# zju-pi/diff-sampler

Measured on AMD Instinct MI355X. Metric: images/sec (whole node) at NFE=10, EDM CIFAR-10, higher is better.
Workload: dtype fp32; 1 GPU; EDM CIFAR-10 32x32 SongUNet (55.7M params), DPM-Solver++(2M) logSNR NFE=10, batch 256/GPU; launch=eager

## Files before the change

### diff_sampler_amd/csrc/conv3x3_thin.hip

```cpp
#include "igemm_common.h"

namespace igemm {
namespace {

template <int CTRL>
__device__ __forceinline__ float thin_dpp_add(float v) {
    return v + __builtin_bit_cast(float, __builtin_amdgcn_update_dpp(0, __builtin_bit_cast(int, v), CTRL, 0xf, 0xf, false));
}

template <int NORM, bool UPD>
__global__ void __launch_bounds__(256, 4) conv3x3_thin_kernel(const KParams p, const ds_update_args u) {
    extern __shared__ __attribute__((aligned(16))) float smem_thin[];
    f32x4* wl = reinterpret_cast<f32x4*>(smem_thin);
    const int tid = threadIdx.x, lane = tid & 63, wave = tid >> 6;
    const int C = p.c0, S = C / 32;
    for (int i = tid; i < 9 * S * 32; i += 256) {
        const int j = i & 7, q = (i >> 3) & 3, rest = i >> 5;
        const int tap = rest / S, step = rest - tap * S;
        const float* b = p.b + (size_t)(step * 9 + tap) * 32 + j * 4 + q;
        wl[i] = f32x4{b[0], b[(size_t)p.ldb], b[2 * (size_t)p.ldb], b[3 * (size_t)p.ldb]};
    }
    __syncthreads();
    const int R = p.mtiles;
    const int mb = blockIdx.x * (32 * R) + wave * (8 * R);
    if (mb >= p.M) return;
    const int img = mb / p.HW;
    const int g = lane >> 3, j = lane & 7;
    const float* coef = NORM ? p.norm + (size_t)img * 3 * C + j * 4 : nullptr;
    const float scale = p.scale;
    f32x4 bias = {0.f, 0.f, 0.f, 0.f};
    if (p.colbias) {
#pragma unroll
        for (int n = 0; n < 4; ++n) bias[n] = n < p.N ? p.colbias[n] : 0.f;
    }
#pragma unroll 1
    for (int round = 0; round < R; ++round) {
        const int m = mb + round * 8 + g;
        const int pim = m - img * p.HW;
        const int y = pim / p.W, x = pim - y * p.W;
        const float* src[9]; float keep[9];
#pragma unroll
        for (int t = 0; t < 9; ++t) {
            const int yy = y + t / 3 - 1, xx = x + t % 3 - 1;
            const bool ok = (unsigned)yy < (unsigned)p.H && (unsigned)xx < (unsigned)p.W;
            src[t] = p.a0 + (size_t)(ok ? (img * p.H + yy) * p.W + xx : m) * p.lda0 + j * 4;
            keep[t] = ok ? 1.f : 0.f;
        }
        f32x4 acc = {0.f, 0.f, 0.f, 0.f};
#pragma unroll 1
        for (int s = 0; s < S; ++s) {
            f32x4 mu = {0.f, 0.f, 0.f, 0.f}, ga = mu, be = mu;
            if constexpr (NORM) {
                mu = *reinterpret_cast<const f32x4*>(coef + s * 32);
                ga = *reinterpret_cast<const f32x4*>(coef + C + s * 32);
                be = *reinterpret_cast<const f32x4*>(coef + 2 * C + s * 32);
            }
            constexpr int TG = NORM ? 3 : 9;
#pragma unroll
            for (int t0 = 0; t0 < 9; t0 += TG) {
                f32x4 v[TG];
#pragma unroll
                for (int t = 0; t < TG; ++t) v[t] = *reinterpret_cast<const f32x4*>(src[t0 + t] + s * 32);
#pragma unroll
                for (int t = 0; t < TG; ++t) {
                    f32x4 a = v[t];
                    if constexpr (NORM) {
                        a = (a - mu) * ga + be;
                        if constexpr (NORM == 2) {
#pragma unroll
                            for (int e = 0; e < 4; ++e) a[e] = ds_silu(a[e]);
                        }
                    }
                    a *= keep[t0 + t];
                    const f32x4* wp = wl + (((t0 + t) * S + s) * 4) * 8 + j;
                    acc += a[0] * wp[0] + a[1] * wp[8] + a[2] * wp[16] + a[3] * wp[24];
                }
            }
        }
#pragma unroll
        for (int n = 0; n < 4; ++n) {
            float r = acc[n];
            r = thin_dpp_add<0xB1>(r);
            r = thin_dpp_add<0x4E>(r);
            r = thin_dpp_add<0x141>(r);
            acc[n] = r;
        }
        if (j == 0) {
            DsUpdCoefs k{};
            float cskip = 0.f, cout_ = 0.f;
            if constexpr (UPD) {
                k = ds_upd_load_coefs(u, img);
                cskip = ds_c_skip(k.sig, u.sigma_data); cout_ = ds_c_out(k.sig, u.sigma_data);
            }
#pragma unroll
            for (int n = 0; n < 4; ++n) {
                if (n < p.N) {
                    const float o = (acc[n] + bias[n]) * scale;
                    if (p.out_planar) p.out[((size_t)img * p.N + n) * p.HW + pim] = o;
                    else p.out[(size_t)m * p.ldo + n] = o;
                    if constexpr (UPD) {
                        const size_t off = ((size_t)img * p.N + n) * p.HW + pim;
                        const float x = u.xe[off];
                        const float xb = u.xb != u.xe ? u.xb[off] : x;
                        float mm, xo;
                        ds_upd_element(k, cskip, cout_, true, u.store_d != 0, x, xb, o, u.hist[0] != nullptr, u.hist[0] ? u.hist[0][off] : 0.f,
                                       u.hist[1] != nullptr, u.hist[1] ? u.hist[1][off] : 0.f, u.hist[2] != nullptr, u.hist[2] ? u.hist[2][off] : 0.f, mm, xo);
                        if (u.m_out) u.m_out[off] = mm;
                        if (u.x_out) u.x_out[off] = xo;
                    }
                }
            }
        }
    }
}

}

bool conv3x3_thin_applicable(const KParams& p) {
    if (p.taps != 9 || p.stride > 1 || p.N < 1 || p.N > 4) return false;
    if (p.c0 <= 0 || p.c0 % 32 || p.c1 || p.ec0 || p.ec1) return false;
    if (p.HW != p.H * p.W || p.HW % 64 || p.M % 64) return false;
    if (p.res || p.cbias || p.rowbias || p.stats || p.act != DS_ACT_NONE || p.splits > 1) return false;
    if (p.norm && p.norm_act != DS_ACT_NONE && p.norm_act != DS_ACT_SILU) return false;
    if (p.nrows_b < 4) return false;
    if (9 * p.c0 * 16 > 150 * 1024) return false;
    return true;
}

static bool thin_update_on(const KParams& p) { return p.upd && (p.upd->x_out || p.upd->m_out); }

int conv3x3_thin_check_update(const KParams& p) {
    if (!thin_update_on(p)) return DS_OK;
    const ds_update_args& u = *p.upd;
    if (!p.out_planar || !u.xe || !u.xb || !u.raw || u.afs || u.f_ld != 0) return DS_E_ARG;
    if (u.c != p.N || (long long)u.n * u.h * u.w != (long long)p.M || u.h * u.w != p.HW) return DS_E_ARG;
    if (u.coefs && u.coef_rows != 1 && u.coef_rows != u.n) return DS_E_ARG;
    return DS_OK;
}

int launch_conv3x3_thin(KParams& p, hipStream_t stream) {
    const int smem = 9 * p.c0 * 16;
    int rounds = 8;
    while (rounds > 1 && (p.M + 32 * rounds - 1) / (32 * rounds) < 512) rounds >>= 1;
    p.mtiles = rounds;
    const unsigned blocks = (unsigned)((p.M + 32 * rounds - 1) / (32 * rounds));
    const bool upd = thin_update_on(p);
    ds_update_args u{};
    if (upd) u = *p.upd;
#define DST_LAUNCH(NORM_, UPD_)                                                                                    \
    do {                                                                                                           \
        DS_ENSURE_DYN_LDS((&conv3x3_thin_kernel<NORM_, UPD_>), 160 * 1024);                                        \
        hipLaunchKernelGGL((conv3x3_thin_kernel<NORM_, UPD_>), dim3(blocks), dim3(256), smem, stream, p, u);       \
    } while (0)
    if (p.norm && p.norm_act == DS_ACT_SILU) { if (upd) DST_LAUNCH(2, true); else DST_LAUNCH(2, false); }
    else if (p.norm) { if (upd) DST_LAUNCH(1, true); else DST_LAUNCH(1, false); }
    else { if (upd) DST_LAUNCH(0, true); else DST_LAUNCH(0, false); }
#undef DST_LAUNCH
    DS_CHECK_LAUNCH();
    return DS_OK;
}

}
```

Baseline: 513.2 images/sec.

## Stage activated input halo tile in LDS for thin 3x3 conv with prefetch

Restructures the thin-output 3x3 conv kernel so each block loads its input tile plus halo once per 32-channel step into LDS. The norm/SiLU activation is applied once per staged element instead of once per tap, and the next step's global loads are prefetched into registers while the current step computes. The round count becomes a template parameter, so accumulators for all rounds stay in registers. Previously each pixel reloaded and re-normalized its nine neighbours from global memory. In exchange it needs more LDS, lowers launch bounds occupancy from 4 to 2 blocks, adds two barriers per channel step, and adds geometry code that must handle row and image boundaries, including a slower fallback when a tile spans two images.

```diff
diff --git a/diff_sampler_amd/csrc/conv3x3_thin.hip b/diff_sampler_amd/csrc/conv3x3_thin.hip
--- a/diff_sampler_amd/csrc/conv3x3_thin.hip
+++ b/diff_sampler_amd/csrc/conv3x3_thin.hip
@@ -8,82 +8,165 @@
     return v + __builtin_bit_cast(float, __builtin_amdgcn_update_dpp(0, __builtin_bit_cast(int, v), CTRL, 0xf, 0xf, false));
 }
 
-template <int NORM, bool UPD>
-__global__ void __launch_bounds__(256, 4) conv3x3_thin_kernel(const KParams p, const ds_update_args u) {
+constexpr int THIN_NI = 12;
+
+__host__ __device__ inline void thin_geometry(int H, int W, int R, int& nc, int& narrow, int& cells) {
+    const int TP = 32 * R, HW = H * W;
+    const int rows = TP % W == 0 ? TP / W : W % TP == 0 ? 1 : (TP + W - 2) / W + 1;
+    const int imgs = HW % TP == 0 ? 1 : TP % HW == 0 ? TP / HW : (TP + HW - 2) / HW + 1;
+    narrow = W % TP == 0 && W > TP;
+    nc = narrow ? TP + 2 : W + 2;
+    cells = (rows + 2 * imgs) * nc;
+}
+
+template <int NORM, bool UPD, int R>
+__global__ void __launch_bounds__(256, 2) conv3x3_thin_kernel(const KParams p, const ds_update_args u) {
     extern __shared__ __attribute__((aligned(16))) float smem_thin[];
-    f32x4* wl = reinterpret_cast<f32x4*>(smem_thin);
     const int tid = threadIdx.x, lane = tid & 63, wave = tid >> 6;
     const int C = p.c0, S = C / 32;
+    f32x4* wl = reinterpret_cast<f32x4*>(smem_thin);
+    f32x4* hal = wl + 9 * S * 32;
+    const int g = lane >> 3, j = lane & 7;
+    constexpr int TP = 32 * R;
+    const int NC = p.WP, HP2 = p.H + 2;
+    const int mb0 = blockIdx.x * TP;
+    const int mlast = (mb0 + TP < p.M ? mb0 + TP : p.M) - 1;
+    const int img0 = mb0 / p.HW, imgL = mlast / p.HW;
+    const int pim0 = mb0 - img0 * p.HW, y0 = pim0 / p.W, x0 = pim0 - y0 * p.W;
+    const int yL = (mlast - imgL * p.HW) / p.W;
+    const int cb = p.nimg ? x0 - 1 : -1;
+    const int prb = img0 * HP2 + y0;
+    const int nitems = (imgL * HP2 + yL + 3 - prb) * NC * 8;
+    const bool multi = imgL != img0;
+    const int pb = mb0 - x0 - p.W;
+    const float* a_base = p.a0 + (long long)pb * p.lda0;
+    auto item_src = [&](int it, unsigned& off, int& im) __attribute__((always_inline)) {
+        const int cell = it >> 3, row = cell / NC, col = cell - row * NC;
+        const int pr = prb + row;
+        im = pr / HP2;
+        const int yy = pr - im * HP2 - 1, xx = cb + col;
+        const bool ok = it < nitems && (unsigned)yy < (unsigned)p.H && (unsigned)xx < (unsigned)p.W;
+        off = (unsigned)(((ok ? (im * p.H + yy) * p.W + xx : mb0) - pb) * p.lda0 + j * 4);
+        return ok;
+    };
+    auto load_quad = [&](unsigned off, int s) __attribute__((always_inline)) {
+        return *reinterpret_cast<const f32x4*>(reinterpret_cast<const char*>(a_base + s * 32) + (size_t)(off * 4u));
+    };
+    unsigned off[THIN_NI], okm = 0;
+#pragma unroll
+    for (int i = 0; i < THIN_NI; ++i) {
+        int im;
+        if (item_src(i * 256 + tid, off[i], im)) okm |= 1u << i;
+    }
+    f32x4 v[THIN_NI];
+    f32x4 mu = {0.f, 0.f, 0.f, 0.f}, ga = mu, be = mu;
+    auto load_coefs = [&](int im, int s) __attribute__((always_inline)) {
+        if constexpr (NORM) {
+            const float* cf = p.norm + (size_t)im * 3 * C + j * 4 + s * 32;
+            mu = *reinterpret_cast<const f32x4*>(cf);
+            ga = *reinterpret_cast<const f32x4*>(cf + C);
+            be = *reinterpret_cast<const f32x4*>(cf + 2 * C);
+        }
+    };
+    auto prefetch = [&](int s) __attribute__((always_inline)) {
+        if (multi) return;
+#pragma unroll
+        for (int i = 0; i < THIN_NI; ++i)
+            if (i * 256 < nitems) v[i] = load_quad(off[i], s);
+        load_coefs(img0, s);
+    };
+    auto activate = [&](f32x4 a) __attribute__((always_inline)) {
+        if constexpr (NORM) {
+            a = (a - mu) * ga + be;
+            if constexpr (NORM == 2) {
+#pragma unroll
+                for (int e = 0; e < 4; ++e) a[e] = ds_silu(a[e]);
+            }
+        }
+        return a;
+    };
+    const f32x4 zero4 = {0.f, 0.f, 0.f, 0.f};
+    auto stage = [&](int s) __attribute__((always_inline)) {
+        DS_RACE_SKEW(wave);
+        if (!multi) {
+#pragma unroll
+            for (int i = 0; i < THIN_NI; ++i) {
+                if (i * 256 >= nitems) break;
+                const int it = i * 256 + tid;
+                const f32x4 a = activate(v[i]);
+                if (it < nitems) hal[it] = (okm >> i) & 1u ? a : zero4;
+            }
+        }
+        for (int it = (multi ? 0 : THIN_NI * 256) + tid; it < nitems; it += 256) {
+            unsigned o_; int im;
+            const bool ok = item_src(it, o_, im);
+            const f32x4 a = load_quad(o_, s);
+            if (multi) load_coefs(im, s);
+            hal[it] = ok ? activate(a) : zero4;
+        }
+    };
+    prefetch(0);
+    DS_RACE_SKEW(wave);
     for (int i = tid; i < 9 * S * 32; i += 256) {
-        const int j = i & 7, q = (i >> 3) & 3, rest = i >> 5;
+        const int jj = i & 7, q = (i >> 3) & 3, rest = i >> 5;
         const int tap = rest / S, step = rest - tap * S;
-        const float* b = p.b + (size_t)(step * 9 + tap) * 32 + j * 4 + q;
+        const float* b = p.b + (size_t)(step * 9 + tap) * 32 + jj * 4 + q;
         wl[i] = f32x4{b[0], b[(size_t)p.ldb], b[2 * (size_t)p.ldb], b[3 * (size_t)p.ldb]};
     }
-    __syncthreads();
-    const int R = p.mtiles;
-    const int mb = blockIdx.x * (32 * R) + wave * (8 * R);
-    if (mb >= p.M) return;
-    const int img = mb / p.HW;
-    const int g = lane >> 3, j = lane & 7;
-    const float* coef = NORM ? p.norm + (size_t)img * 3 * C + j * 4 : nullptr;
+    const int mbw = mb0 + wave * (8 * R);
+    const bool active = mbw < p.M;
+    int cc[R];
+#pragma unroll
+    for (int r = 0; r < R; ++r) {
+        const int m = active ? mbw + r * 8 + g : mb0;
+        const int img = m / p.HW, pim = m - img * p.HW, y = pim / p.W, x = pim - y * p.W;
+        cc[r] = ((img * HP2 + y + 1 - prb) * NC + (x - cb)) * 8 + j;
+    }
+    f32x4 acc[R];
+#pragma unroll
+    for (int r = 0; r < R; ++r) acc[r] = zero4;
+#pragma unroll 1
+    for (int s = 0; s < S; ++s) {
+        stage(s);
+        __syncthreads();
+        if (s + 1 < S) prefetch(s + 1);
+        if (active) {
+#pragma unroll
+            for (int t = 0; t < 9; ++t) {
+                const f32x4* wp = wl + ((t * S + s) * 4) * 8 + j;
+                const f32x4 w0 = wp[0], w1 = wp[8], w2 = wp[16], w3 = wp[24];
+                const int d = ((t / 3 - 1) * NC + (t % 3 - 1)) * 8;
+constexpr int RG = R < 4 ? R : 4;
+#pragma unroll
+                for (int r0 = 0; r0 < R; r0 += RG) {
+                    f32x4 a[RG];
+#pragma unroll
+                    for (int r = 0; r < RG; ++r) a[r] = hal[cc[r0 + r] + d];
+#pragma unroll
+                    for (int r = 0; r < RG; ++r) acc[r0 + r] += a[r][0] * w0 + a[r][1] * w1 + a[r][2] * w2 + a[r][3] * w3;
+                }
+            }
+        }
+        if (s + 1 < S) __syncthreads();
+    }
+    if (!active) return;
     const float scale = p.scale;
-    f32x4 bias = {0.f, 0.f, 0.f, 0.f};
+    f32x4 bias = zero4;
     if (p.colbias) {
 #pragma unroll
         for (int n = 0; n < 4; ++n) bias[n] = n < p.N ? p.colbias[n] : 0.f;
     }
-#pragma unroll 1
-    for (int round = 0; round < R; ++round) {
-        const int m = mb + round * 8 + g;
-        const int pim = m - img * p.HW;
-        const int y = pim / p.W, x = pim - y * p.W;
-        const float* src[9]; float keep[9];
-#pragma unroll
-        for (int t = 0; t < 9; ++t) {
-            const int yy = y + t / 3 - 1, xx = x + t % 3 - 1;
-            const bool ok = (unsigned)yy < (unsigned)p.H && (unsigned)xx < (unsigned)p.W;
-            src[t] = p.a0 + (size_t)(ok ? (img * p.H + yy) * p.W + xx : m) * p.lda0 + j * 4;
-            keep[t] = ok ? 1.f : 0.f;
-        }
-        f32x4 acc = {0.f, 0.f, 0.f, 0.f};
-#pragma unroll 1
-        for (int s = 0; s < S; ++s) {
-            f32x4 mu = {0.f, 0.f, 0.f, 0.f}, ga = mu, be = mu;
-            if constexpr (NORM) {
-                mu = *reinterpret_cast<const f32x4*>(coef + s * 32);
-                ga = *reinterpret_cast<const f32x4*>(coef + C + s * 32);
-                be = *reinterpret_cast<const f32x4*>(coef + 2 * C + s * 32);
-            }
-            constexpr int TG = NORM ? 3 : 9;
-#pragma unroll
-            for (int t0 = 0; t0 < 9; t0 += TG) {
-                f32x4 v[TG];
-#pragma unroll
-                for (int t = 0; t < TG; ++t) v[t] = *reinterpret_cast<const f32x4*>(src[t0 + t] + s * 32);
-#pragma unroll
-                for (int t = 0; t < TG; ++t) {
-                    f32x4 a = v[t];
-                    if constexpr (NORM) {
-                        a = (a - mu) * ga + be;
-                        if constexpr (NORM == 2) {
-#pragma unroll
-                            for (int e = 0; e < 4; ++e) a[e] = ds_silu(a[e]);
-                        }
-                    }
-                    a *= keep[t0 + t];
-                    const f32x4* wp = wl + (((t0 + t) * S + s) * 4) * 8 + j;
-                    acc += a[0] * wp[0] + a[1] * wp[8] + a[2] * wp[16] + a[3] * wp[24];
-                }
-            }
-        }
+#pragma unroll
+    for (int r = 0; r < R; ++r) {
+        const int m = mbw + r * 8 + g;
+        const int img = m / p.HW, pim = m - img * p.HW;
 #pragma unroll
         for (int n = 0; n < 4; ++n) {
-            float r = acc[n];
-            r = thin_dpp_add<0xB1>(r);
-            r = thin_dpp_add<0x4E>(r);
-            r = thin_dpp_add<0x141>(r);
-            acc[n] = r;
+            float q = acc[r][n];
+            q = thin_dpp_add<0xB1>(q);
+            q = thin_dpp_add<0x4E>(q);
+            q = thin_dpp_add<0x141>(q);
+            acc[r][n] = q;
         }
         if (j == 0) {
             DsUpdCoefs k{};
@@ -95,18 +178,18 @@
 #pragma unroll
             for (int n = 0; n < 4; ++n) {
                 if (n < p.N) {
-                    const float o = (acc[n] + bias[n]) * scale;
+                    const float o = (acc[r][n] + bias[n]) * scale;
                     if (p.out_planar) p.out[((size_t)img * p.N + n) * p.HW + pim] = o;
                     else p.out[(size_t)m * p.ldo + n] = o;
                     if constexpr (UPD) {
-                        const size_t off = ((size_t)img * p.N + n) * p.HW + pim;
-                        const float x = u.xe[off];
-                        const float xb = u.xb != u.xe ? u.xb[off] : x;
+                        const size_t off_ = ((size_t)img * p.N + n) * p.HW + pim;
+                        const float x = u.xe[off_];
+                        const float xb = u.xb != u.xe ? u.xb[off_] : x;
                         float mm, xo;
-                        ds_upd_element(k, cskip, cout_, true, u.store_d != 0, x, xb, o, u.hist[0] != nullptr, u.hist[0] ? u.hist[0][off] : 0.f,
-                                       u.hist[1] != nullptr, u.hist[1] ? u.hist[1][off] : 0.f, u.hist[2] != nullptr, u.hist[2] ? u.hist[2][off] : 0.f, mm, xo);
-                        if (u.m_out) u.m_out[off] = mm;
-                        if (u.x_out) u.x_out[off] = xo;
+                        ds_upd_element(k, cskip, cout_, true, u.store_d != 0, x, xb, o, u.hist[0] != nullptr, u.hist[0] ? u.hist[0][off_] : 0.f,
+                                       u.hist[1] != nullptr, u.hist[1] ? u.hist[1][off_] : 0.f, u.hist[2] != nullptr, u.hist[2] ? u.hist[2][off_] : 0.f, mm, xo);
+                        if (u.m_out) u.m_out[off_] = mm;
+                        if (u.x_out) u.x_out[off_] = xo;
                     }
                 }
             }
@@ -114,6 +197,19 @@
     }
 }
 
+}
+
+static int thin_tile(const KParams& p, int& rounds, int& halo_cols, int& narrow) {
+    constexpr int LDS_MAX = 160 * 1024;
+    int cells;
+    rounds = 8;
+    while (rounds > 2 && (p.M + 32 * rounds - 1) / (32 * rounds) < 512) rounds >>= 1;
+    for (;; rounds >>= 1) {
+        thin_geometry(p.H, p.W, rounds, halo_cols, narrow, cells);
+        const int smem = 9 * p.c0 * 16 + cells * 128;
+        if (rounds == 2) return smem <= LDS_MAX ? smem : 0;
+        if (cells * 8 <= THIN_NI * 256 && smem <= LDS_MAX) return smem;
+    }
 }
 
 bool conv3x3_thin_applicable(const KParams& p) {
@@ -123,8 +219,8 @@
     if (p.res || p.cbias || p.rowbias || p.stats || p.act != DS_ACT_NONE || p.splits > 1) return false;
     if (p.norm && p.norm_act != DS_ACT_NONE && p.norm_act != DS_ACT_SILU) return false;
     if (p.nrows_b < 4) return false;
-    if (9 * p.c0 * 16 > 150 * 1024) return false;
-    return true;
+    int rounds, halo_cols, narrow;
+    return thin_tile(p, rounds, halo_cols, narrow) > 0;
 }
 
 static bool thin_update_on(const KParams& p) { return p.upd && (p.upd->x_out || p.upd->m_out); }
@@ -139,23 +235,30 @@
 }
 
 int launch_conv3x3_thin(KParams& p, hipStream_t stream) {
-    const int smem = 9 * p.c0 * 16;
-    int rounds = 8;
-    while (rounds > 1 && (p.M + 32 * rounds - 1) / (32 * rounds) < 512) rounds >>= 1;
-    p.mtiles = rounds;
+    int rounds, halo_cols, narrow;
+    const int smem = thin_tile(p, rounds, halo_cols, narrow);
+    if (smem <= 0) return DS_E_ARG;
+    p.mtiles = rounds; p.WP = halo_cols; p.nimg = narrow;
     const unsigned blocks = (unsigned)((p.M + 32 * rounds - 1) / (32 * rounds));
     const bool upd = thin_update_on(p);
     ds_update_args u{};
     if (upd) u = *p.upd;
+#define DST_LAUNCH_R(NORM_, UPD_, R_)                                                                              \
+    do {                                                                                                           \
+        DS_ENSURE_DYN_LDS((&conv3x3_thin_kernel<NORM_, UPD_, R_>), 160 * 1024);                                    \
+        hipLaunchKernelGGL((conv3x3_thin_kernel<NORM_, UPD_, R_>), dim3(blocks), dim3(256), smem, stream, p, u);   \
+    } while (0)
 #define DST_LAUNCH(NORM_, UPD_)                                                                                    \
     do {                                                                                                           \
-        DS_ENSURE_DYN_LDS((&conv3x3_thin_kernel<NORM_, UPD_>), 160 * 1024);                                        \
-        hipLaunchKernelGGL((conv3x3_thin_kernel<NORM_, UPD_>), dim3(blocks), dim3(256), smem, stream, p, u);       \
+        if (rounds == 8) DST_LAUNCH_R(NORM_, UPD_, 8);                                                             \
+        else if (rounds == 4) DST_LAUNCH_R(NORM_, UPD_, 4);                                                        \
+        else DST_LAUNCH_R(NORM_, UPD_, 2);                                                                         \
     } while (0)
     if (p.norm && p.norm_act == DS_ACT_SILU) { if (upd) DST_LAUNCH(2, true); else DST_LAUNCH(2, false); }
     else if (p.norm) { if (upd) DST_LAUNCH(1, true); else DST_LAUNCH(1, false); }
     else { if (upd) DST_LAUNCH(0, true); else DST_LAUNCH(0, false); }
 #undef DST_LAUNCH
+#undef DST_LAUNCH_R
     DS_CHECK_LAUNCH();
     return DS_OK;
 }
```

After: 514.5 images/sec, median of 6. About the same (+0.3%).
